# rlvc/FEALESS

Measured on AMD Instinct MI355X. Metric: frames/sec (640x480 RGB-D x N templates, 20 ICP iters), higher is better.
Workload: dtype u8

## Files before the change

fealess_amd/csrc/fl_context.hip:

```cpp
#include "fl_internal.h"
#include <stdlib.h>
#include <stdarg.h>
#include <string.h>
#include <algorithm>

int fl_set_error(fl_context *ctx, int code, const char *fmt, ...)
{
  if (ctx) {
    va_list ap;
    va_start(ap, fmt);
    vsnprintf(ctx->err, sizeof(ctx->err), fmt, ap);
    va_end(ap);
  }
  return code;
}

int fl_scratch(fl_context *ctx, size_t bytes, void **out)
{
  if (int rc = fl_context_join(ctx)) return rc;
  if (bytes > ctx->scratch_bytes) {
    if (ctx->scratch) {
      FL_HIP(ctx, hipStreamSynchronize(ctx->stream));
      FL_HIP(ctx, hipFree(ctx->scratch));
      ctx->scratch = nullptr;
      ctx->scratch_bytes = 0;
    }
    size_t nb = fl_align(bytes + bytes / 4, 1 << 20);
    FL_HIP(ctx, hipMalloc(&ctx->scratch, nb));
    ctx->scratch_bytes = nb;
  }
  *out = ctx->scratch;
  return FL_OK;
}

int fl_pinned(fl_context *ctx, size_t bytes, void **out)
{
  if (int rc = fl_context_join(ctx)) return rc;
  if (bytes > ctx->pinned_bytes) {
    if (ctx->pinned) {
      FL_HIP(ctx, hipStreamSynchronize(ctx->stream));
      FL_HIP(ctx, hipHostFree(ctx->pinned));
      ctx->pinned = nullptr;
      ctx->pinned_bytes = 0;
    }
    size_t nb = fl_align(bytes, 1 << 16);
    FL_HIP(ctx, hipHostMalloc(&ctx->pinned, nb, hipHostMallocDefault));
    ctx->pinned_bytes = nb;
  }
  *out = ctx->pinned;
  return FL_OK;
}

int fl_context_join(fl_context *ctx)
{
  if (!ctx->icp_pending) return FL_OK;
  ctx->icp_pending = false;
  FL_HIP(ctx, hipStreamWaitEvent(ctx->stream, ctx->ev_icp_tail, 0));
  return FL_OK;
}

int fl_context_sync_all(fl_context *ctx)
{
  FL_HIP(ctx, hipStreamSynchronize(ctx->stream));
  if (ctx->icp_stream) FL_HIP(ctx, hipStreamSynchronize(ctx->icp_stream));
  ctx->icp_pending = false;
  return FL_OK;
}

int fl_icp_stream(fl_context *ctx, hipStream_t *out)
{
  const long mode = ctx->opt.pipeline_icp;
  if (ctx->icp_stream && ctx->icp_stream_mode != mode) {
    FL_HIP(ctx, hipStreamSynchronize(ctx->icp_stream));
    FL_HIP(ctx, hipStreamDestroy(ctx->icp_stream));
    ctx->icp_stream = nullptr;
  }
  if (!ctx->icp_stream) {
    int least = 0, greatest = 0;
    FL_HIP(ctx, hipDeviceGetStreamPriorityRange(&least, &greatest));
    FL_HIP(ctx, hipStreamCreateWithPriority(&ctx->icp_stream, hipStreamNonBlocking, mode == 2 ? greatest : (mode == 3 ? least : 0)));
    ctx->icp_stream_mode = mode;
  }
  if (!ctx->ev_icp_tail) FL_HIP(ctx, hipEventCreateWithFlags(&ctx->ev_icp_tail, hipEventDisableTiming));
  *out = ctx->icp_stream;
  return FL_OK;
}

extern "C" int fl_abi_version(void) { return FL_ABI_VERSION; }

struct FlOptionName { const char *name, *env; long fl_context::Options::*field; bool hex; long lo, hi; };
static const FlOptionName fl_option_names[] = {
  {"scan_prune", "FL_SCAN_PRUNE", &fl_context::Options::scan_prune, false, 0, 1},
  {"scan_prune_mid", "FL_SCAN_PRUNE_MID", &fl_context::Options::scan_prune_mid, true, -1, 0xFF},
  {"icp_wide", "FL_ICP_WIDE", &fl_context::Options::icp_wide, false, -1, 1},
  {"icp_occ", "FL_ICP_OCC", &fl_context::Options::icp_occ, false, 0, 5},
  {"icp_order", "FL_ICP_ORDER", &fl_context::Options::icp_order, false, 0, 1},
  {"icp_wg_per_cu", "FL_ICP_WG_PER_CU", &fl_context::Options::icp_wg_per_cu, false, 0, 3},
  {"eager_frontend", "FL_EAGER_FRONTEND", &fl_context::Options::eager_frontend, false, 0, 1},
  {"dev_poison", "FL_DEV_POISON", &fl_context::Options::dev_poison, false, 0, 1},
  {"ws_pad", "FL_DEV_WS_PAD", &fl_context::Options::ws_pad, false, 0, 16l << 20},
  {"pipeline_icp", "FL_PIPELINE_ICP", &fl_context::Options::pipeline_icp, false, 0, 3},
  {"frontend_chunk_rows", "FL_FRONTEND_CHUNK_ROWS", &fl_context::Options::frontend_chunk_rows, false, 0, 60 * 1024},
  {"scan_run", "FL_SCAN_RUN", &fl_context::Options::scan_run, false, 0, 64},
  {"refine_lds", "FL_REFINE_LDS", &fl_context::Options::refine_lds, false, 0, 2},
  {"refine_lds_bytes", "FL_REFINE_LDS_BYTES", &fl_context::Options::refine_lds_bytes, false, 0, FL_REFINE_LDS_BYTES},
  {"verify_fused", "FL_VERIFY_FUSED", &fl_context::Options::verify_fused, false, 0, 1},
  {"verify_fused_px", "FL_VERIFY_FUSED_PX", &fl_context::Options::verify_fused_px, false, 0, FL_VERIFY_FUSED_PX},
};

static bool fl_option_valid(const FlOptionName &o, long v)
{
  if (v < o.lo || v > o.hi) return false;
  if (o.field == &fl_context::Options::frontend_chunk_rows) return v % 60 == 0;
  if (o.field == &fl_context::Options::verify_fused_px) return v == 0 || v >= FL_WAVE;
  return o.field != &fl_context::Options::icp_occ || v == 0 || v >= 4;
}

extern "C" int fl_context_create(int device, fl_context **out)
{
  if (!out) return FL_ERR_INVALID;
  *out = nullptr;
  int n = 0;
  if (hipGetDeviceCount(&n) != hipSuccess || n <= 0) return FL_ERR_NO_DEVICE;
  if (device < 0 || device >= n) return FL_ERR_INVALID;
  fl_context *ctx = new fl_context();
  ctx->device = device;
  if (hipSetDevice(device) != hipSuccess ||
      hipStreamCreateWithFlags(&ctx->own_stream, hipStreamNonBlocking) != hipSuccess) {
    delete ctx;
    return FL_ERR_HIP;
  }
  ctx->stream = ctx->own_stream;
  {
    hipDeviceProp_t prop;
    if (hipGetDeviceProperties(&prop, device) == hipSuccess && prop.multiProcessorCount > 0) ctx->cus = prop.multiProcessorCount;
  }
  for (const FlOptionName &o : fl_option_names)
    if (const char *e = getenv(o.env)) {
      const long v = o.hex ? (long)strtoul(e, nullptr, 16) : atol(e);
      if (fl_option_valid(o, v)) ctx->opt.*(o.field) = v;
    }
  *out = ctx;
  return FL_OK;
}

extern "C" void *fl_context_get_stream(fl_context *ctx) { return ctx ? (void *)ctx->stream : nullptr; }
extern "C" int fl_context_get_device(const fl_context *ctx) { return ctx ? ctx->device : -1; }
extern "C" fl_context *fl_detector_get_context(fl_detector *det) { return det ? det->ctx : nullptr; }

extern "C" int fl_context_set_option(fl_context *ctx, const char *name, long value)
{
  if (!ctx || !name) return FL_ERR_INVALID;
  for (const FlOptionName &o : fl_option_names)
    if (!strcmp(name, o.name)) {
      if (!fl_option_valid(o, value)) return fl_set_error(ctx, FL_ERR_INVALID, "option '%s': %ld is out of range", name, value);
      ctx->opt.*(o.field) = value;
      return FL_OK;
    }
  return fl_set_error(ctx, FL_ERR_INVALID, "unknown option '%s'", name);
}

extern "C" int fl_context_get_option(const fl_context *ctx, const char *name, long *value)
{
  if (!ctx || !name || !value) return FL_ERR_INVALID;
  for (const FlOptionName &o : fl_option_names)
    if (!strcmp(name, o.name)) { *value = ctx->opt.*(o.field); return FL_OK; }
  return FL_ERR_INVALID;
}

static void context_release(fl_context *ctx)
{
  if (ctx->device < 0) { delete ctx; return; }
  (void)hipSetDevice(ctx->device);
  (void)fl_context_sync_all(ctx);
  if (ctx->icp_stream) (void)hipStreamDestroy(ctx->icp_stream);
  if (ctx->ev_icp_tail) (void)hipEventDestroy(ctx->ev_icp_tail);
  if (ctx->scratch) (void)hipFree(ctx->scratch);
  if (ctx->pinned) (void)hipHostFree(ctx->pinned);
  if (ctx->own_stream) (void)hipStreamDestroy(ctx->own_stream);
  delete ctx;
}

extern "C" void fl_context_destroy(fl_context *ctx)
{
  if (!ctx) return;
  if (ctx->detectors > 0) { ctx->destroy_pending = true; return; }
  context_release(ctx);
}

extern "C" const char *fl_last_error(const fl_context *ctx) { return ctx ? ctx->err : "null context"; }

extern "C" int fl_context_set_stream(fl_context *ctx, void *hip_stream)
{
  if (!ctx) return FL_ERR_INVALID;
  if (int rc = fl_context_sync_all(ctx)) return rc;
  ctx->stream = hip_stream ? (hipStream_t)hip_stream : ctx->own_stream;
  return FL_OK;
// ... 543 lines not shown
```

fealess_amd/csrc/fl_internal.h:

```cpp
#pragma once
#include <hip/hip_runtime.h>
#include <cmath>
#include <stdint.h>
#include <stdio.h>
#include <string>
#include <vector>
#include "../../include/fealess_hip.h"

#define FL_WAVE 64

struct fl_context {
  int device = 0;
  hipStream_t own_stream = nullptr;
  hipStream_t stream = nullptr;
  hipStream_t icp_stream = nullptr;
  long icp_stream_mode = 0;
  hipEvent_t ev_icp_tail = nullptr;
  bool icp_pending = false;
  char err[512] = {0};
  void *scratch = nullptr;
  size_t scratch_bytes = 0;
  void *pinned = nullptr;
  size_t pinned_bytes = 0;
  int cus = 256;
  struct Options {
    long scan_prune = 1;
    long scan_prune_mid = -1;
    long icp_wide = -1;
    long icp_occ = 0;
    long icp_order = 1;
    long icp_wg_per_cu = 0;
    long eager_frontend = 0;
    long dev_poison = 0;
    long ws_pad = 0;
    long pipeline_icp = 3;
    long frontend_chunk_rows = 0;
    long scan_run = 0;
    long refine_lds = 0;
    long refine_lds_bytes = 0;
    long verify_fused = 0;
    long verify_fused_px = 0;
  } opt;
  bool verify_fused_attr = false;
  int detectors = 0;
  bool destroy_pending = false;
};

int fl_set_error(fl_context *ctx, int code, const char *fmt, ...);
int fl_scratch(fl_context *ctx, size_t bytes, void **out);
int fl_pinned(fl_context *ctx, size_t bytes, void **out);
int fl_context_join(fl_context *ctx);
int fl_context_sync_all(fl_context *ctx);
int fl_icp_stream(fl_context *ctx, hipStream_t *out);

#define FL_HIP(ctx, call)                                                                  \
  do {                                                                                     \
    hipError_t e_ = (call);                                                                \
    if (e_ != hipSuccess)                                                                  \
      return fl_set_error((ctx), FL_ERR_HIP, "%s:%d: %s -> %s", __FILE__, __LINE__, #call, \
                          hipGetErrorString(e_));                                          \
  } while (0)

static inline size_t fl_align(size_t v, size_t a) { return (v + a - 1) / a * a; }
static inline bool fl_finite_all(const float *p, size_t n)
{
  for (size_t i = 0; i < n; ++i)
    if (!std::isfinite(p[i])) return false;
  return true;
}

#define FL_MAX_LEVELS 4
#define FL_MAX_MODALITIES 2
#define FL_MAX_FEATURES 63

struct FlScanHdr {
  int32_t P;
  int32_t off_begin;
  int32_t n_pad;
  int32_t nf;
};
struct FlScanItem {
  uint32_t off0[8];
  int32_t g;
  uint32_t chunk_nf;
  struct {
    int32_t P;
    int32_t off_begin;
    uint32_t npad_nf;
  } mod[FL_MAX_MODALITIES];
};
static_assert(sizeof(FlScanItem) == 64 && FL_MAX_MODALITIES == 2, "a dword per lane of a 16-lane load");
#define FL_SCAN_OFF_PAD 8
void fl_build_scan_items(const std::vector<FlScanHdr> &hdr, int n_pyr, int M, int WH, uint32_t zero_off, std::vector<uint32_t> &scan_off,
                         std::vector<FlScanItem> &items);
struct FlFineFeat {
  int16_t x, y;
  int16_t qx, qy;
  uint8_t gx, gy;
  uint8_t label, pad;
};
struct FlFineHdr {
  int32_t feat_begin, feat_count;
  int32_t width, height;
};
struct FlFineBox {
  int16_t x0, y0, x1, y1;
};
struct FlPyrInfo {
  int32_t class_idx, template_id;
  int32_t off_x0, off_y0, width0, height0;
// ... 336 lines not shown
```

fealess_amd/csrc/fl_linemod.hip:

```cpp
#include "fl_internal.h"
#include <limits.h>
#include <string.h>
#include <algorithm>
#include <type_traits>

__global__ __launch_bounds__(256) void k_build_lm_generic(FlPlanes pl, int n_mod, int w, int h, int T, int W, int WH, uint32_t stride)
{
  const int p = blockIdx.x * 256 + threadIdx.x;
  const int gi = blockIdx.y;
  const int frame = blockIdx.z / n_mod, m = blockIdx.z - frame * n_mod;
  const uint8_t *q = pl.in + (size_t)frame * pl.in_stride + pl.in_off[m];
  uint8_t *out = pl.out + (size_t)frame * pl.out_stride + pl.out_off[m];
  if (p >= WH) return;
  const int gy = gi / T, gx = gi - gy * T;
  const int yt = p / W, xt = p - yt * W;
  const int y = yt * T + gy, x = xt * T + gx;
  unsigned b = 0;
  const int rmax = min(T, h - y), cmax = min(T, w - x);
  for (int r = 0; r < rmax; ++r) {
    const uint8_t *row = q + (size_t)(y + r) * w + x;
    for (int c = 0; c < cmax; ++c) b |= row[c];
  }
  const unsigned bb = b | (b << 8);
#pragma unroll
// ... 314 lines not shown
{
  if (w % 4 == 0 && T <= 8 && T >= 2 && planes_aligned(pl, n_mod, 4)) {
    int k = 4;
    for (; k > 1 && (size_t)2 * (k * T + T - 1) * (w + 16) > 60 * 1024; --k) {}
    const size_t lds = (size_t)(2 * k * T + T - 1) * (w + 16);
    if ((size_t)2 * (k * T + T - 1) * (w + 16) <= 64 * 1024) {
      SpreadArgs a{pl, tiles, tiles_stride, w, h, T, k * T};
      const bool v16 = !tiles && w % 16 == 0 && planes_aligned(pl, n_mod, 16);
      dim3 grid((h + a.RS - 1) / a.RS, n_mod, n_frames);
      hipLaunchKernelGGL(FL_PICK_T(k_spread, T, v16), grid, dim3(256), lds, ctx->stream, a);
      FL_HIP(ctx, hipGetLastError());
      return FL_OK;
    }
  }
  dim3 grid((w + 63) / 64, (h + 3) / 4, n_frames * n_mod);
  hipLaunchKernelGGL(k_spread_generic, grid, dim3(256), 0, ctx->stream, pl, n_mod, w, h, T);
  FL_HIP(ctx, hipGetLastError());
  return FL_OK;
}

static size_t build_lm_lds(int w, int W, int T, int HB)
{
  return std::max<size_t>(((size_t)HB * (w + 16) + 15) & ~(size_t)15, 2048) + (size_t)T * HB * W;
}

#define FL_LM_LDS (20 * 1024)
#define FL_LM_BLOCKS 1024
#define FL_LM_RUN 256
static int build_lm_band(int n_frames, int n_mod, int w, int h, int T)
{
  if (T < 2 || T > 8 || w % 4 != 0) return 0;
  const int W = w / T, H = h / T;
  if (W < 4 || W % 4 != 0 || H < 1) return 0;
  int HB = H;
  while (HB > 1 && build_lm_lds(w, W, T, HB) > FL_LM_LDS) --HB;
  if (build_lm_lds(w, W, T, HB) > 64 * 1024) return 0;
  const long blocks = (long)n_frames * n_mod * T;
  if (blocks < FL_LM_BLOCKS) {
    const int bands = (int)((FL_LM_BLOCKS + blocks - 1) / blocks);
    HB = min(HB, max(max(H / bands, (FL_LM_RUN + W - 1) / W), 1));
  }
  int step = 1;
  while ((step * W) % 16 != 0) step *= 2;
  if (HB < H && HB >= step) HB -= HB % step;
  return HB;
}
extern "C" int fl_dev_build_lm_band(int n_frames, int n_mod, int w, int h, int T) { return build_lm_band(n_frames, n_mod, w, h, T); }

int fl_launch_build_lm(fl_context *ctx, const FlPlanes &pl, int n_mod, int n_frames, int w, int h, int T)
{
  const int W = w / T, H = h / T, WH = W * H;
  const uint32_t stride = (uint32_t)fl_lm_label_stride(w, h, T);
  const int HB = planes_aligned(pl, n_mod, 4) ? build_lm_band(n_frames, n_mod, w, h, T) : 0;
  if (HB) {
    BuildLmArgs a{pl, n_frames, w, h, T, W, H, HB, (H + HB - 1) / HB, 0, stride};
    a.out16 = WH % 16 == 0 && (a.nbands == 1 || (HB * W) % 16 == 0) && planes_aligned(pl, n_mod, 16);
    const bool v16 = w % 16 == 0 && planes_aligned(pl, n_mod, 16);
    dim3 grid((unsigned)(8 * ((n_frames + 7) / 8) * T * a.nbands), n_mod, 1);
    hipLaunchKernelGGL(FL_PICK_T(k_build_lm, T, v16), grid, dim3(256), build_lm_lds(w, W, T, HB), ctx->stream, a);
    FL_HIP(ctx, hipGetLastError());
    return FL_OK;
  }
  dim3 grid((WH + 255) / 256, T * T, n_frames * n_mod);
  hipLaunchKernelGGL(k_build_lm_generic, grid, dim3(256), 0, ctx->stream, pl, n_mod, w, h, T, W, WH, stride);
  FL_HIP(ctx, hipGetLastError());
  return FL_OK;
}

struct ScanArgs {
  const FlScanItem *items;
  int n_items;
  const uint32_t *offs;
  const uint8_t *enabled;
  uint8_t *ws;
  size_t ws_stride;
  size_t lm_off[FL_MAX_MODALITIES];
  size_t off_count, off_cand;
  int M, W, WH, T, cap;
  int bpf, n_frames;
  int run, wave_step, item_step;
  float threshold;
  int prune;
  unsigned prune_mid;
  uint16_t *dbg;
  int dbg_first, dbg_count;
};

typedef unsigned int u32x4 __attribute__((ext_vector_type(4)));
typedef unsigned short u16x2 __attribute__((ext_vector_type(2)));
__device__ __forceinline__ u16x2 pk_bytes_max(uint32_t a)
{
  const uint32_t lo = a & 0x00FF00FFu, hi = (a >> 8) & 0x00FF00FFu;
  return __builtin_elementwise_max(__builtin_bit_cast(u16x2, lo), __builtin_bit_cast(u16x2, hi));
}
__device__ __forceinline__ uint4 ld16(const uint8_t *p)
{
  uint4 v;
  __builtin_memcpy(&v, p, 16);
  return v;
}
#define FL_CONST_AS __attribute__((address_space(4)))
__device__ __forceinline__ uint32_t sload1(const void *p) { return *(const FL_CONST_AS uint32_t *)(uintptr_t)p; }
__device__ __forceinline__ uint32_t rl(uint32_t v, int l) { return (uint32_t)__builtin_amdgcn_readlane((int)v, l); }

#ifndef FL_SCAN_PRUNE_MID
#define FL_SCAN_PRUNE_MID 0x7Fu
#endif
#ifndef FL_SCAN_OFFSETS_AHEAD
#define FL_SCAN_OFFSETS_AHEAD 1
#endif
#ifndef FL_SCAN_WPE
#define FL_SCAN_WPE 5
#endif
#ifndef FL_SCAN_WPE_PRUNED
#define FL_SCAN_WPE_PRUNED 6
#endif
template <int WPE>
__global__ __launch_bounds__(256) __attribute__((amdgpu_waves_per_eu(WPE, WPE))) void k_scan(ScanArgs a)
{
  const int wave = threadIdx.x >> 6, lane = threadIdx.x & 63;
  const int xcd = blockIdx.x & 7, q = blockIdx.x >> 3;
  const int frame = xcd + 8 * (q / a.bpf);
  if (frame >= a.n_frames) return;
  int it = __builtin_amdgcn_readfirstlane(((q % a.bpf) * 4 + wave) * a.wave_step);
  if (it >= a.n_items) return;
  const int l7 = lane & 7;
  auto request_item = [&](int idx) {
    const uint32_t *p = lane < 16 ? (const uint32_t *)(a.items + idx) + lane : (const uint32_t *)(a.enabled + (idx & ~3));
    return *p;
  };
  uint32_t rec = request_item(it);
  const uint8_t *lm[FL_MAX_MODALITIES];
  for (int m = 0; m < FL_MAX_MODALITIES; ++m) lm[m] = a.ws + (size_t)frame * a.ws_stride + a.lm_off[m];
  const float thr100 = a.threshold / 100.f;
  const unsigned lane_off = (unsigned)lane * 16u;
  const int dbg_first = a.dbg_first;
  const unsigned dbg_count = (unsigned)a.dbg_count;
  const FL_CONST_AS ScanArgs *ka = (const FL_CONST_AS ScanArgs *)__builtin_amdgcn_kernarg_segment_ptr();

  auto scan_item = [&](const uint32_t r) {
    const int g = (int)rl(r, 8), chunk = (int)(rl(r, 9) & 0xFFFFu), nf_all = (int)(rl(r, 9) >> 16);
    const int rP[FL_MAX_MODALITIES] = {(int)rl(r, 10), (int)rl(r, 13)}, rB[FL_MAX_MODALITIES] = {(int)rl(r, 11), (int)rl(r, 14)};
    const uint32_t rN[FL_MAX_MODALITIES] = {rl(r, 12), rl(r, 15)};
    const int j0 = chunk * 1024 + lane * 16;

    uint32_t tot[16];
#pragma unroll
    for (int i = 0; i < 16; ++i) tot[i] = 0;
    const int prune_threshold = (int)(2 * nf_all + thr100 * (2 * nf_all) + 0.5f);
    const bool tapped = (unsigned)(g - dbg_first) < dbg_count;
    const bool prune = a.prune && !tapped;
    const unsigned mid = prune ? a.prune_mid : 0u;
    uint32_t ov = r;
    int o_at = (rN[0] & 0xFFFFu) ? rB[0] : -1;
    int nf = 0;
#pragma unroll
    for (int m = 0; m < FL_MAX_MODALITIES; ++m) {
      if (m >= a.M) break;
      const int P = rP[m], off_begin = rB[m], n_pad = (int)(rN[m] & 0xFFFFu), h_nf = (int)(rN[m] >> 16);
      uint32_t mx_tot = 0;
      if (prune && m > 0) {
#pragma unroll
        for (int i = 0; i < 16; ++i) mx_tot = max(mx_tot, tot[i]);
        if (__ballot((int)mx_tot + 4 * (nf_all - nf) > prune_threshold) == 0ull) return;
      }
      nf += h_nf;
      if (chunk * 1024 >= P) continue;
      const uint8_t *lm_u = lm[m] + chunk * 1024;
      const __amdgpu_buffer_rsrc_t rsrc = __builtin_amdgcn_make_buffer_rsrc((void *)(lm_u - 4), 0, 0x7FFFFFFF, 0x00020000);
      uint32_t a0 = 0, a1 = 0, a2 = 0, a3 = 0;
      const unsigned lm_mis = (unsigned)(size_t)lm_u & 3u;
      const int lanes_on = min(64, ((P - chunk * 1024 + 15) >> 4) + 1);
      const bool on = lane < lanes_on;
      const int next_begin = rB[m + 1 < FL_MAX_MODALITIES ? m + 1 : m];
      for (int k = 0; k < n_pad; k += 8) {
        const int at = off_begin + k;
        if (o_at != at) ov = a.offs[at + l7];
        const int nxt_at = k + 8 < n_pad ? at + 8 : next_begin;
        const uint32_t nxt = a.offs[nxt_at + l7];
        uint32_t o[8];
#pragma unroll
        for (int u = 0; u < 8; ++u) o[u] = rl(ov, u);
        if (on) {
        uint4 v[8];
        uint32_t e[8];
        unsigned mis_all = 0;
#pragma unroll
        for (int u = 0; u < 8; ++u) {
          const unsigned off = o[u];
          const unsigned mis_u = (lm_mis + off) & 3u;
          mis_all |= mis_u << (4 * u);
          const u32x4 ld = __builtin_amdgcn_raw_buffer_load_b128(rsrc, lane_off, off - mis_u + 4u, 0);
          v[u] = make_uint4(ld.x, ld.y, ld.z, ld.w);
          const uint32_t tail = sload1(lm_u + off - mis_u + 1024);
          e[u] = (uint32_t)__builtin_amdgcn_update_dpp((int)tail, (int)v[u].x, 0x130, 0xF, 0xF, false);
        }
#pragma unroll
        for (int u = 0; u < 8; ++u) {
          const unsigned mis_u = (mis_all >> (4 * u)) & 3u;
          a0 += __builtin_amdgcn_alignbyte(v[u].y, v[u].x, mis_u);
          a1 += __builtin_amdgcn_alignbyte(v[u].z, v[u].y, mis_u);
          a2 += __builtin_amdgcn_alignbyte(v[u].w, v[u].z, mis_u);
          a3 += __builtin_amdgcn_alignbyte(e[u], v[u].w, mis_u);
        }
        asm volatile("" :: "v"(nxt));
        }
        ov = nxt;
        o_at = FL_SCAN_OFFSETS_AHEAD ? nxt_at : -1;
        if ((mid >> (k >> 3)) & 1u) {
          const u16x2 b0 = pk_bytes_max(a0), b1 = pk_bytes_max(a1), b2 = pk_bytes_max(a2), b3 = pk_bytes_max(a3);
          const u16x2 bm = __builtin_elementwise_max(__builtin_elementwise_max(b0, b1), __builtin_elementwise_max(b2, b3));
          const int part = (int)max(bm.x, bm.y);
          const int left = nf_all - nf + max(0, h_nf - (k + 8));
          if (__ballot((int)mx_tot + part + 4 * left > prune_threshold) == 0ull) return;
        }
      }
      const uint32_t acc[4] = {a0, a1, a2, a3};
#pragma unroll
      for (int i = 0; i < 16; ++i) {
        uint32_t byte = (acc[i >> 2] >> ((i & 3) * 8)) & 0xFFu;
        tot[i] += (j0 + i < P) ? byte : 0u;
      }
    }
    if (tapped) {
      const FL_CONST_AS ScanArgs *kr = ka;
      asm volatile("" : "+s"(kr));
      const int WH = kr->WH;
      uint16_t *d = kr->dbg + ((size_t)frame * dbg_count + (g - dbg_first)) * WH;
#pragma unroll
      for (int i = 0; i < 16; ++i)
        if (j0 + i < WH) d[j0 + i] = (uint16_t)tot[i];
    }
    const int raw_threshold = (int)(2 * nf + thr100 * (2 * nf) + 0.5f);
    uint32_t mx = 0;
#pragma unroll
    for (int i = 0; i < 16; ++i) mx = max(mx, tot[i]);
    if ((int)mx <= raw_threshold) return;
    const FL_CONST_AS ScanArgs *kr = ka;
    asm volatile("" : "+s"(kr));
    const int W = kr->W, WH = kr->WH, T = kr->T, cap = kr->cap;
    uint8_t *ws = kr->ws + (size_t)frame * kr->ws_stride;
    int *count = (int *)(ws + kr->off_count);
    FlCand *cand = (FlCand *)(ws + kr->off_cand);
    const int offset = T / 2 + (T % 2 - 1);
#pragma unroll
    for (int i = 0; i < 16; ++i) {
      const int raw = (int)tot[i];
      const int j = j0 + i;
      if (raw > raw_threshold && j < WH) {
        const int rr = j / W, c = j - rr * W;
        const int idx = atomicAdd(count, 1);
        if (idx < cap) {
          FlCand cd;
          cd.x = c * T + offset;
          cd.y = rr * T + offset;
          cd.g = g;
          cd.sim = (raw * 100.f) / (4 * nf) + 0.5f;
          cand[idx] = cd;
        }
      }
    }
  };

  const int it_end = min(a.n_items, it + a.run * a.item_step);
  for (;;) {
    const uint32_t cur = rec;
    const bool cur_on = ((rl(cur, 16) >> ((it & 3) * 8)) & 0xFFu) != 0;
    const int nx = it + a.item_step;
    const bool more = nx < it_end;
    const int nxc = more ? nx : it;
    rec = request_item(nxc);
    if (cur_on) scan_item(cur);
    if (!more) break;
    it = nx;
  }
}

__device__ __noinline__ uint32_t refine_slow_path(const uint8_t *sp, bool in, int xt0, int yt0, int gx, int gy, int T,
                                                  int W, int H, int w)
{
  uint32_t out = 0;
  const int g0 = gy * T + gx, TT = T * T;
  for (int c = 0; c < 4; ++c) {
    int xx = xt0 + c, yy = yt0, gg = g0;
    const int wx = xx >= W ? xx / W : 0;
    xx -= wx * W;
    yy += wx;
    const int wy = yy >= H ? yy / H : 0;
    yy -= wy * H;
    gg += wy;
    if (in && gg < TT) {
      const int ggy = gg / T, ggx = gg - ggy * T;
      out |= (uint32_t)sp[(size_t)(yy * T + ggy) * w + (size_t)(xx * T + ggx)] << (8 * c);
    }
  }
  return out;
}

struct RefineArgs {
  const FlFineHdr *hdr;
  const FlFineFeat *feat;
  uint8_t *ws;
  size_t ws_stride;
  size_t spread_off[FL_MAX_MODALITIES];
  size_t off_count, off_cand;
  int M, Lm1, level, w, h, T, W, H, cap;
  float threshold;
};

struct RefinePlace { int x, y, offset_x, offset_y; };

__device__ __forceinline__ RefinePlace refine_place(const RefineArgs &a, const FlFineHdr *hdr, int cx, int cy, int T)
{
  const int border = 8 * T;
  const int max_x = a.w - hdr[0].width - border;
  const int max_y = a.h - hdr[0].height - border;
  RefinePlace p;
  p.x = min(max(cx * 2 + 1, border), max_x);
  p.y = min(max(cy * 2 + 1, border), max_y);
  p.offset_x = (p.x / T - 8) * T;
// ... 455 lines not shown
  for (int i = threadIdx.x; i < n; i += blockDim.x) {
    const FlCand c = cand[i];
    if (c.g >= 0) {
      const FlPyrInfo pi = a.pyr[c.g];
      Key128 k;
      k.hi = ((unsigned long long)__float_as_uint(c.sim) << 32) | (unsigned)(0x7FFFFFFF - pi.template_id);
      k.lo = ((unsigned long long)(0xFFFF - pi.class_idx) << 32) | ((unsigned long long)(0xFFFF - (c.y + 32768)) << 16) |
             (unsigned long long)(0xFFFF - (c.x + 32768));
      const int slot = atomicAdd(&s_n, 1);
      gkeys[slot] = k;
    }
  }
  __syncthreads();
  const int nl = s_n;
  int n2 = 1;
  while (n2 < nl) n2 <<= 1;
  const Key128 zero = {0ull, 0ull};
  Key128 *keys;
  if (n2 <= FL_SORT_LDS_KEYS) {
    for (int i = threadIdx.x; i < n2; i += blockDim.x) lds_keys[i] = i < nl ? gkeys[i] : zero;
    keys = lds_keys;
    bitonic_desc<true>(keys, n2);
  } else {
    for (int i = nl + threadIdx.x; i < n2; i += blockDim.x) gkeys[i] = zero;
    keys = gkeys;
    bitonic_desc<false>(keys, n2);
  }
  for (int base = 0; base < nl; base += blockDim.x) {
    const int i = base + threadIdx.x;
    int flag = 0;
    Key128 k = zero;
    if (i < nl) {
      k = keys[i];
      if (i == 0) flag = 1;
      else {
        const Key128 p = keys[i - 1];
        flag = !((k.hi >> 32) == (p.hi >> 32) && k.lo == p.lo);
      }
    }
    s_scan[threadIdx.x] = flag;
    __syncthreads();
    for (int d = 1; d < (int)blockDim.x; d <<= 1) {
      int v = threadIdx.x >= d ? s_scan[threadIdx.x - d] : 0;
      __syncthreads();
      s_scan[threadIdx.x] += v;
      __syncthreads();
    }
    const int pos = s_base + s_scan[threadIdx.x] - flag;
    if (flag) {
      fl_match m;
      m.similarity = __uint_as_float((unsigned)(k.hi >> 32));
      m.template_id = 0x7FFFFFFF - (int)(k.hi & 0xFFFFFFFFu);
      m.class_idx = 0xFFFF - (int)(k.lo >> 32);
      m.y = (0xFFFF - (int)((k.lo >> 16) & 0xFFFF)) - 32768;
      m.x = (0xFFFF - (int)(k.lo & 0xFFFF)) - 32768;
      out[pos] = m;
    }
    __syncthreads();
    if (threadIdx.x == blockDim.x - 1) s_base += s_scan[threadIdx.x];
    __syncthreads();
  }
  if (threadIdx.x == 0) {
    counters[1] = s_base;
    counters[2] = n_raw > a.cap ? 1 : 0;
  }
}

#ifndef FL_SCAN_RUN_AUTO
#define FL_SCAN_RUN_AUTO 8
#endif
#ifndef FL_SCAN_STRIDED
#define FL_SCAN_STRIDED 1
#endif
#define FL_SCAN_FILL 4
static int fl_scan_run(const fl_context *ctx, int items, int n_frames)
{
  if (ctx->opt.scan_run) return (int)ctx->opt.scan_run;
  const long need = (long)FL_SCAN_FILL * ctx->cus * 4 * (ctx->opt.scan_prune ? FL_SCAN_WPE_PRUNED : FL_SCAN_WPE);
  int run = FL_SCAN_RUN_AUTO;
  while (run > 1 && (long)n_frames * ((items + run - 1) / run) < need) run /= 2;
  return run;
}

#ifndef FL_REFINE_LDS_FRAMES_PER_CU
#define FL_REFINE_LDS_FRAMES_PER_CU 1
#endif
static bool fl_refine_use_lds(const fl_detector *det, int level, int n_frames, long *budget)
{
  const fl_context *ctx = det->ctx;
  *budget = ctx->opt.refine_lds_bytes ? ctx->opt.refine_lds_bytes : (long)FL_REFINE_LDS_BYTES;
  if (ctx->opt.refine_lds == 1 || det->refine_window_max[level] > *budget) return false;
  return ctx->opt.refine_lds == 2 || n_frames >= FL_REFINE_LDS_FRAMES_PER_CU * ctx->cus;
}

extern "C" int fl_dev_refine_pitch(int width, int T) { return fl_refine_pitch(width, fl_refine_qmask(T)); }
extern "C" int fl_dev_refine_plan(const int32_t *rects, int n, int max_len, long budget, int T, int32_t *uni)
{
  FlRect u;
  const int len = fl_refine_plan(rects, n, max_len, budget, fl_refine_qmask(T), &u);
  if (uni) { uni[0] = u.x0; uni[1] = u.y0; uni[2] = u.x1; uni[3] = u.y1; }
  return len;
}
extern "C" int fl_dev_refine_kernel(const fl_detector *det, int level)
{
  return det && level >= 0 && level < det->L - 1 ? det->refine_ran[level] : -1;
}
extern "C" long fl_dev_refine_window_max(const fl_detector *det, int level)
{
  return det && level >= 0 && level < det->L - 1 ? det->refine_window_max[level] : -1;
}

static int launch_scan_refine_sort(fl_detector *det, int n_frames, float threshold, uint16_t *dbg, int dbg_first,
                                   int dbg_count)
{
  fl_context *ctx = det->ctx;
  const int L = det->L, M = det->M;
  {
    const FlLevelGeom &g = det->geom[L - 1];
    ScanArgs a;
    a.offs = det->d_scan_off;
    a.enabled = det->d_item_enabled;
    a.ws = det->d_ws;
    a.ws_stride = det->ws_stride;
    for (int m = 0; m < FL_MAX_MODALITIES; ++m) a.lm_off[m] = g.lm_off[m < M ? m : 0];
    a.off_count = det->off_count;
    a.off_cand = det->off_cand;
    a.M = M;
    a.W = g.W;
    a.WH = g.WH;
    a.T = g.T;
    a.cap = det->cap;
    a.threshold = threshold;
    a.prune = ctx->opt.scan_prune != 0;
    a.prune_mid = ctx->opt.scan_prune_mid >= 0 ? (unsigned)ctx->opt.scan_prune_mid : FL_SCAN_PRUNE_MID;
    a.dbg = dbg;
    a.dbg_first = dbg_first;
    a.dbg_count = dbg ? dbg_count : 0;
    a.items = det->d_scan_items;
    a.n_items = det->n_scan_items;
    const int items = det->n_scan_items;
    if (items > 0) {
      a.run = fl_scan_run(ctx, items, n_frames);
      const int waves = (items + a.run - 1) / a.run;
      a.bpf = (waves + 3) / 4;
#if FL_SCAN_STRIDED
      a.wave_step = 1;
      a.item_step = a.bpf * 4;
#else
      a.wave_step = a.run;
      a.item_step = 1;
#endif
      a.n_frames = n_frames;
      dim3 grid((unsigned)(a.bpf * ((n_frames + 7) / 8) * 8));
      if (a.prune) hipLaunchKernelGGL(k_scan<FL_SCAN_WPE_PRUNED>, grid, dim3(256), 0, ctx->stream, a);
      else hipLaunchKernelGGL(k_scan<FL_SCAN_WPE>, grid, dim3(256), 0, ctx->stream, a);
      FL_HIP(ctx, hipGetLastError());
    }
  }
  if (det->have_times) FL_HIP(ctx, hipEventRecord(det->ev[3], ctx->stream));
  for (int l = L - 2; l >= 0; --l) {
    const FlLevelGeom &g = det->geom[l];
    RefineArgs a;
    const bool lazy_level = det->lazy;
    a.hdr = det->d_fine_hdr;
    a.feat = det->d_fine_feat;
    a.ws = det->d_ws;
    a.ws_stride = det->ws_stride;
    for (int m = 0; m < FL_MAX_MODALITIES; ++m) a.spread_off[m] = g.spread_off[m < M ? m : 0];
    a.off_count = det->off_count;
    a.off_cand = det->off_cand;
    a.M = M;
    a.Lm1 = L - 1;
    a.level = l;
    a.w = g.w;
    a.h = g.h;
    a.T = g.T;
    a.W = g.W;
    a.H = g.H;
    a.cap = det->cap;
    a.threshold = threshold;
    if (lazy_level) {
      if (det->have_times) FL_HIP(ctx, hipEventRecord(det->ev[8 + 2 * l], ctx->stream));
      hipLaunchKernelGGL(k_mark_tiles, dim3(n_frames), dim3(256), 0, ctx->stream, a, det->off_tiles);
      FL_HIP(ctx, hipGetLastError());
      int rc = fl_launch_lazy_level(det, n_frames, l);
      if (rc) return rc;
      if (det->have_times) FL_HIP(ctx, hipEventRecord(det->ev[9 + 2 * l], ctx->stream));
    }
    long budget;
    if (fl_refine_use_lds(det, l, n_frames, &budget)) {
      const uint32_t qmask = fl_refine_qmask(g.T);
      const dim3 grid(n_frames), block(256);
      switch (g.T) {
      case 4: hipLaunchKernelGGL(k_refine_lds<4>, grid, block, 0, ctx->stream, a, det->d_fine_box, (int)budget, qmask); break;
      case 5: hipLaunchKernelGGL(k_refine_lds<5>, grid, block, 0, ctx->stream, a, det->d_fine_box, (int)budget, qmask); break;
      case 8: hipLaunchKernelGGL(k_refine_lds<8>, grid, block, 0, ctx->stream, a, det->d_fine_box, (int)budget, qmask); break;
      default: hipLaunchKernelGGL(k_refine_lds<0>, grid, block, 0, ctx->stream, a, det->d_fine_box, (int)budget, qmask); break;
      }
      det->refine_ran[l] = 2;
#ifdef FL_REFINE_STATS
      {
        unsigned long long st[4], zero[4] = {0, 0, 0, 0};
        FL_HIP(ctx, hipStreamSynchronize(ctx->stream));
        FL_HIP(ctx, hipMemcpyFromSymbol(st, HIP_SYMBOL(d_refine_stats), sizeof(st)));
        FL_HIP(ctx, hipMemcpyToSymbol(HIP_SYMBOL(d_refine_stats), zero, sizeof(zero)));
        fprintf(stderr, "k_refine_lds level %d: %d frames, %llu with candidates, %.2f groups per such frame, %.0f bytes staged per group, "
                "%.2f candidates per group\n", l, n_frames, st[0], st[0] ? (double)st[1] / st[0] : 0.0, st[1] ? (double)st[2] / st[1] : 0.0,
                st[1] ? (double)st[3] / st[1] : 0.0);
      }
#endif
    } else {
      dim3 grid(n_frames >= 64 ? 4 : (n_frames >= 8 ? 32 : 256), n_frames);
      hipLaunchKernelGGL(k_refine, grid, dim3(256), 0, ctx->stream, a);
      det->refine_ran[l] = 1;
    }
    FL_HIP(ctx, hipGetLastError());
  }
  if (det->have_times) FL_HIP(ctx, hipEventRecord(det->ev[4], ctx->stream));
  {
    SortArgs a;
    a.pyr = det->d_pyr;
    a.ws = det->d_ws;
    a.ws_stride = det->ws_stride;
    a.off_count = det->off_count;
    a.off_cand = det->off_cand;
    a.off_keys = det->off_keys;
    a.off_match = det->off_match;
    a.cap = det->cap;
    hipLaunchKernelGGL(k_sort_unique, dim3(n_frames), dim3(1024), 0, ctx->stream, a);
    FL_HIP(ctx, hipGetLastError());
  }
  if (det->have_times) FL_HIP(ctx, hipEventRecord(det->ev[5], ctx->stream));
  return FL_OK;
}

int fl_launch_match_core(fl_detector *det, int n_frames, float threshold)
{
  fl_context *ctx = det->ctx;
  if (det->set_busy[det->set]) {
// ... 731 lines not shown
```

Measured before the change: 88210.

## Prune scan per lane and check bound at finer feature steps

The LINEMOD scan kernel now keeps a per-lane alive mask, so lanes whose candidates can no longer reach the threshold stop issuing loads instead of waiting for the whole wave to fail. Feature accumulation can also be split into steps of 2 or 4 offsets with a bound check after each, chosen by frame count (step 4 at 256 frames or more). Tail scalar loads are skipped when the last lane is dead. This cuts memory loads for hopeless candidates, at the cost of extra ballots and branches, more template variants, and some optional stats instrumentation.

```diff
diff --git a/fealess_amd/csrc/fl_context.hip b/fealess_amd/csrc/fl_context.hip
--- a/fealess_amd/csrc/fl_context.hip
+++ b/fealess_amd/csrc/fl_context.hip
@@ -92,6 +92,8 @@
 static const FlOptionName fl_option_names[] = {
   {"scan_prune", "FL_SCAN_PRUNE", &fl_context::Options::scan_prune, false, 0, 1},
   {"scan_prune_mid", "FL_SCAN_PRUNE_MID", &fl_context::Options::scan_prune_mid, true, -1, 0xFF},
+  {"scan_prune_lanes", "FL_SCAN_PRUNE_LANES", &fl_context::Options::scan_prune_lanes, false, 0, 1},
+  {"scan_prune_step", "FL_SCAN_PRUNE_STEP", &fl_context::Options::scan_prune_step, false, 0, 8},
   {"icp_wide", "FL_ICP_WIDE", &fl_context::Options::icp_wide, false, -1, 1},
   {"icp_occ", "FL_ICP_OCC", &fl_context::Options::icp_occ, false, 0, 5},
   {"icp_order", "FL_ICP_ORDER", &fl_context::Options::icp_order, false, 0, 1},
@@ -113,6 +115,7 @@
   if (v < o.lo || v > o.hi) return false;
   if (o.field == &fl_context::Options::frontend_chunk_rows) return v % 60 == 0;
   if (o.field == &fl_context::Options::verify_fused_px) return v == 0 || v >= FL_WAVE;
+  if (o.field == &fl_context::Options::scan_prune_step) return v == 0 || v == 2 || v == 4 || v == 8;
   return o.field != &fl_context::Options::icp_occ || v == 0 || v >= 4;
 }
 
diff --git a/fealess_amd/csrc/fl_internal.h b/fealess_amd/csrc/fl_internal.h
--- a/fealess_amd/csrc/fl_internal.h
+++ b/fealess_amd/csrc/fl_internal.h
@@ -26,6 +26,8 @@
   struct Options {
     long scan_prune = 1;
     long scan_prune_mid = -1;
+    long scan_prune_lanes = 1;
+    long scan_prune_step = 0;
     long icp_wide = -1;
     long icp_occ = 0;
     long icp_order = 1;
diff --git a/fealess_amd/csrc/fl_linemod.hip b/fealess_amd/csrc/fl_linemod.hip
--- a/fealess_amd/csrc/fl_linemod.hip
+++ b/fealess_amd/csrc/fl_linemod.hip
@@ -420,6 +420,7 @@
   float threshold;
   int prune;
   unsigned prune_mid;
+  int prune_lanes;
   uint16_t *dbg;
   int dbg_first, dbg_count;
 };
@@ -453,9 +454,24 @@
 #ifndef FL_SCAN_WPE_PRUNED
 #define FL_SCAN_WPE_PRUNED 6
 #endif
-template <int WPE>
+#ifndef FL_SCAN_STEP
+#define FL_SCAN_STEP 4
+#endif
+#ifndef FL_SCAN_TAIL_ALWAYS
+#define FL_SCAN_TAIL_ALWAYS 0
+#endif
+#ifdef FL_SCAN_STATS
+#define FL_SCAN_STATS_N (4 + 2 * FL_MAX_FEATURES + 1)
+__device__ unsigned long long d_scan_stats[FL_SCAN_STATS_N];
+#define FL_SCAN_STAT(i, v) do { if (lane == 0) atomicAdd(&d_scan_stats[i], (unsigned long long)(v)); } while (0)
+#else
+#define FL_SCAN_STAT(i, v) do { } while (0)
+#endif
+template <int N> struct ScanInt { static constexpr int value = N; };
+template <int WPE, int STEP>
 __global__ __launch_bounds__(256) __attribute__((amdgpu_waves_per_eu(WPE, WPE))) void k_scan(ScanArgs a)
 {
+  static_assert(STEP == 8 || STEP == 4 || STEP == 2, "a group of eight offsets is cut into equal parts");
   const int wave = threadIdx.x >> 6, lane = threadIdx.x & 63;
   const int xcd = blockIdx.x & 7, q = blockIdx.x >> 3;
   const int frame = xcd + 8 * (q / a.bpf);
@@ -489,6 +505,15 @@
     const bool tapped = (unsigned)(g - dbg_first) < dbg_count;
     const bool prune = a.prune && !tapped;
     const unsigned mid = prune ? a.prune_mid : 0u;
+    const bool by_lane = prune && a.prune_lanes;
+    uint64_t alive = ~0ull;
+    auto still = [&](bool reachable) {
+      const uint64_t b = __ballot(reachable) & alive;
+      alive = by_lane || b == 0ull ? b : ~0ull;
+      return alive != 0ull;
+    };
+    [[maybe_unused]] int f_done = 0;
+    FL_SCAN_STAT(0, 1);
     uint32_t ov = r;
     int o_at = (rN[0] & 0xFFFFu) ? rB[0] : -1;
     int nf = 0;
@@ -500,7 +525,10 @@
       if (prune && m > 0) {
 #pragma unroll
         for (int i = 0; i < 16; ++i) mx_tot = max(mx_tot, tot[i]);
-        if (__ballot((int)mx_tot + 4 * (nf_all - nf) > prune_threshold) == 0ull) return;
+        if (!still((int)mx_tot + 4 * (nf_all - nf) > prune_threshold)) {
+          FL_SCAN_STAT(4 + f_done, 1);
+          return;
+        }
       }
       nf += h_nf;
       if (chunk * 1024 >= P) continue;
@@ -509,49 +537,84 @@
       uint32_t a0 = 0, a1 = 0, a2 = 0, a3 = 0;
       const unsigned lm_mis = (unsigned)(size_t)lm_u & 3u;
       const int lanes_on = min(64, ((P - chunk * 1024 + 15) >> 4) + 1);
-      const bool on = lane < lanes_on;
+      const uint64_t lanes_mask = lanes_on >= 64 ? ~0ull : (1ull << lanes_on) - 1ull;
       const int next_begin = rB[m + 1 < FL_MAX_MODALITIES ? m + 1 : m];
       for (int k = 0; k < n_pad; k += 8) {
         const int at = off_begin + k;
         if (o_at != at) ov = a.offs[at + l7];
         const int nxt_at = k + 8 < n_pad ? at + 8 : next_begin;
         const uint32_t nxt = a.offs[nxt_at + l7];
-        uint32_t o[8];
-#pragma unroll
-        for (int u = 0; u < 8; ++u) o[u] = rl(ov, u);
-        if (on) {
-        uint4 v[8];
-        uint32_t e[8];
-        unsigned mis_all = 0;
-#pragma unroll
-        for (int u = 0; u < 8; ++u) {
-          const unsigned off = o[u];
-          const unsigned mis_u = (lm_mis + off) & 3u;
-          mis_all |= mis_u << (4 * u);
-          const u32x4 ld = __builtin_amdgcn_raw_buffer_load_b128(rsrc, lane_off, off - mis_u + 4u, 0);
-          v[u] = make_uint4(ld.x, ld.y, ld.z, ld.w);
-          const uint32_t tail = sload1(lm_u + off - mis_u + 1024);
-          e[u] = (uint32_t)__builtin_amdgcn_update_dpp((int)tail, (int)v[u].x, 0x130, 0xF, 0xF, false);
-        }
-#pragma unroll
-        for (int u = 0; u < 8; ++u) {
-          const unsigned mis_u = (mis_all >> (4 * u)) & 3u;
-          a0 += __builtin_amdgcn_alignbyte(v[u].y, v[u].x, mis_u);
-          a1 += __builtin_amdgcn_alignbyte(v[u].z, v[u].y, mis_u);
-          a2 += __builtin_amdgcn_alignbyte(v[u].w, v[u].z, mis_u);
-          a3 += __builtin_amdgcn_alignbyte(e[u], v[u].w, mis_u);
-        }
-        asm volatile("" :: "v"(nxt));
+        auto add_features = [&](auto s0_, auto n_) {
+          constexpr int S0 = decltype(s0_)::value, N = decltype(n_)::value;
+          uint32_t o[N];
+#pragma unroll
+          for (int u = 0; u < N; ++u) o[u] = rl(ov, S0 + u);
+          const uint64_t need = (alive | alive << 1) & lanes_mask;
+          FL_SCAN_STAT(1, N);
+          FL_SCAN_STAT(2, N * __builtin_popcountll(need));
+          const bool tail_on = FL_SCAN_TAIL_ALWAYS || (need >> 63) != 0ull;
+          uint32_t tail[N];
+#pragma unroll
+          for (int u = 0; u < N; ++u) tail[u] = 0u;
+          if (__builtin_amdgcn_inverse_ballot_w64(need)) {
+          uint4 v[N];
+          uint32_t e[N];
+          unsigned mis_all = 0;
+          if (tail_on) {
+#pragma unroll
+            for (int u = 0; u < N; ++u) tail[u] = sload1(lm_u + o[u] - ((lm_mis + o[u]) & 3u) + 1024);
+          }
+#pragma unroll
+          for (int u = 0; u < N; ++u) {
+            const unsigned off = o[u];
+            const unsigned mis_u = (lm_mis + off) & 3u;
+            mis_all |= mis_u << (4 * u);
+            const u32x4 ld = __builtin_amdgcn_raw_buffer_load_b128(rsrc, lane_off, off - mis_u + 4u, 0);
+            v[u] = make_uint4(ld.x, ld.y, ld.z, ld.w);
+            e[u] = (uint32_t)__builtin_amdgcn_update_dpp((int)tail[u], (int)v[u].x, 0x130, 0xF, 0xF, false);
+          }
+#pragma unroll
+          for (int u = 0; u < N; ++u) {
+            const unsigned mis_u = (mis_all >> (4 * u)) & 3u;
+            a0 += __builtin_amdgcn_alignbyte(v[u].y, v[u].x, mis_u);
+            a1 += __builtin_amdgcn_alignbyte(v[u].z, v[u].y, mis_u);
+            a2 += __builtin_amdgcn_alignbyte(v[u].w, v[u].z, mis_u);
+            a3 += __builtin_amdgcn_alignbyte(e[u], v[u].w, mis_u);
+          }
+          if (S0 == 0) asm volatile("" :: "v"(nxt));
+          }
+          f_done += N;
+        };
+        auto reachable = [&](int done) {
+          const u16x2 b0 = pk_bytes_max(a0), b1 = pk_bytes_max(a1), b2 = pk_bytes_max(a2), b3 = pk_bytes_max(a3);
+          const u16x2 bm = __builtin_elementwise_max(__builtin_elementwise_max(b0, b1), __builtin_elementwise_max(b2, b3));
+          const int part = (int)max(bm.x, bm.y);
+          const int left = nf_all - nf + max(0, h_nf - done);
+          if (still((int)mx_tot + part + 4 * left > prune_threshold)) return true;
+          FL_SCAN_STAT(4 + f_done, 1);
+          return false;
+        };
+        const bool chk = (mid >> (k >> 3)) & 1u;
+        if (STEP == 8 || k == 0) {
+          add_features(ScanInt<0>{}, ScanInt<8>{});
+          if (chk && !reachable(k + 8)) return;
+        } else if (STEP == 4) {
+          add_features(ScanInt<0>{}, ScanInt<4>{});
+          if (chk && !reachable(k + 4)) return;
+          add_features(ScanInt<4>{}, ScanInt<4>{});
+          if (chk && !reachable(k + 8)) return;
+        } else {
+          add_features(ScanInt<0>{}, ScanInt<2>{});
+          if (chk && !reachable(k + 2)) return;
+          add_features(ScanInt<2>{}, ScanInt<2>{});
+          if (chk && !reachable(k + 4)) return;
+          add_features(ScanInt<4>{}, ScanInt<2>{});
+          if (chk && !reachable(k + 6)) return;
+          add_features(ScanInt<6>{}, ScanInt<2>{});
+          if (chk && !reachable(k + 8)) return;
         }
         ov = nxt;
         o_at = FL_SCAN_OFFSETS_AHEAD ? nxt_at : -1;
-        if ((mid >> (k >> 3)) & 1u) {
-          const u16x2 b0 = pk_bytes_max(a0), b1 = pk_bytes_max(a1), b2 = pk_bytes_max(a2), b3 = pk_bytes_max(a3);
-          const u16x2 bm = __builtin_elementwise_max(__builtin_elementwise_max(b0, b1), __builtin_elementwise_max(b2, b3));
-          const int part = (int)max(bm.x, bm.y);
-          const int left = nf_all - nf + max(0, h_nf - (k + 8));
-          if (__ballot((int)mx_tot + part + 4 * left > prune_threshold) == 0ull) return;
-        }
       }
       const uint32_t acc[4] = {a0, a1, a2, a3};
 #pragma unroll
@@ -573,7 +636,8 @@
     uint32_t mx = 0;
 #pragma unroll
     for (int i = 0; i < 16; ++i) mx = max(mx, tot[i]);
-    if ((int)mx <= raw_threshold) return;
+    FL_SCAN_STAT(3, 1);
+    if ((int)mx <= raw_threshold || !__builtin_amdgcn_inverse_ballot_w64(alive)) return;
     const FL_CONST_AS ScanArgs *kr = ka;
     asm volatile("" : "+s"(kr));
     const int W = kr->W, WH = kr->WH, T = kr->T, cap = kr->cap;
@@ -1195,6 +1259,15 @@
   return run;
 }
 
+#ifndef FL_SCAN_STEP_FRAMES
+#define FL_SCAN_STEP_FRAMES 256
+#endif
+static int fl_scan_step(const fl_context *ctx, int n_frames)
+{
+  if (ctx->opt.scan_prune_step) return (int)ctx->opt.scan_prune_step;
+  return n_frames >= FL_SCAN_STEP_FRAMES ? FL_SCAN_STEP : 8;
+}
+
 #ifndef FL_REFINE_LDS_FRAMES_PER_CU
 #define FL_REFINE_LDS_FRAMES_PER_CU 1
 #endif
@@ -1246,6 +1319,7 @@
     a.threshold = threshold;
     a.prune = ctx->opt.scan_prune != 0;
     a.prune_mid = ctx->opt.scan_prune_mid >= 0 ? (unsigned)ctx->opt.scan_prune_mid : FL_SCAN_PRUNE_MID;
+    a.prune_lanes = ctx->opt.scan_prune_lanes != 0;
     a.dbg = dbg;
     a.dbg_first = dbg_first;
     a.dbg_count = dbg ? dbg_count : 0;
@@ -1265,9 +1339,26 @@
 #endif
       a.n_frames = n_frames;
       dim3 grid((unsigned)(a.bpf * ((n_frames + 7) / 8) * 8));
-      if (a.prune) hipLaunchKernelGGL(k_scan<FL_SCAN_WPE_PRUNED>, grid, dim3(256), 0, ctx->stream, a);
-      else hipLaunchKernelGGL(k_scan<FL_SCAN_WPE>, grid, dim3(256), 0, ctx->stream, a);
+      if (!a.prune) hipLaunchKernelGGL((k_scan<FL_SCAN_WPE, 8>), grid, dim3(256), 0, ctx->stream, a);
+      else switch (fl_scan_step(ctx, n_frames)) {
+      case 2: hipLaunchKernelGGL((k_scan<FL_SCAN_WPE_PRUNED, 2>), grid, dim3(256), 0, ctx->stream, a); break;
+      case 4: hipLaunchKernelGGL((k_scan<FL_SCAN_WPE_PRUNED, 4>), grid, dim3(256), 0, ctx->stream, a); break;
+      default: hipLaunchKernelGGL((k_scan<FL_SCAN_WPE_PRUNED, 8>), grid, dim3(256), 0, ctx->stream, a); break;
+      }
       FL_HIP(ctx, hipGetLastError());
+#ifdef FL_SCAN_STATS
+      {
+        unsigned long long st[FL_SCAN_STATS_N], zero[FL_SCAN_STATS_N] = {0};
+        FL_HIP(ctx, hipStreamSynchronize(ctx->stream));
+        FL_HIP(ctx, hipMemcpyFromSymbol(st, HIP_SYMBOL(d_scan_stats), sizeof(st)));
+        FL_HIP(ctx, hipMemcpyToSymbol(HIP_SYMBOL(d_scan_stats), zero, sizeof(zero)));
+        fprintf(stderr, "k_scan: %d frames, %llu items, %.2f feature loads and %.1f lane-loads per item, %llu items to their end; ended "
+                "after f features:", n_frames, st[0], st[0] ? (double)st[1] / st[0] : 0.0, st[0] ? (double)st[2] / st[0] : 0.0, st[3]);
+        for (int f = 0; f + 4 < FL_SCAN_STATS_N; ++f)
+          if (st[4 + f]) fprintf(stderr, " %d: %llu", f, st[4 + f]);
+        fprintf(stderr, "\n");
+      }
+#endif
     }
   }
   if (det->have_times) FL_HIP(ctx, hipEventRecord(det->ev[3], ctx->stream));
```

New measurement: 89670, median of 6. 1.02x the previous value.
